# Bardli/RMem_ocu

Hardware: AMD Instinct MI355X
Metric: frames/sec (whole node) 480p VOS, N=8 memory bank (higher is better)
Workload: dtype bf16; 1 GPU; davis17_480p_r50_N8; clip_frames=80, job_clips=64, clip_feeder=static, objects=3, memory_bank=1+7, gap=5, clips_in_flight_per_gpu=24, clips_per_group=8, step_unit=batch, parallelism=clip-parallel x1, weights=synthetic (no checkpoint offline), hipgraphs=True, frames_from=HBM, encoder_lookahead=2

## Files before the change

### include/rmem.h

```cpp
#ifndef RMEM_H_
#define RMEM_H_

#include <stddef.h>

#ifdef __cplusplus
extern "C" {
#endif

#define RMEM_ABI_VERSION 15

int rmem_abi_version(void);
const char* rmem_last_error_string(void);

typedef struct rmem_conv_desc {
  int H, W, Cin;
  int Ho, Wo, Cout;
  int KH, KW, stride, pad;
  int ldo;
  int ldr;
  int ld2;
  int relu;
  int out_f32;
  int res_f32;
  int ldx;
// ... 92 lines not shown
typedef struct rmem_chain_a_desc {
  int L, clips; float eps; int reserved;
  const void* att; float* x;
  const void* w_proj; const float* b_proj; const float* ln2_g; const float* ln2_b; void* curr_v;
  const void* w_q; const float* b_q; void* curr_q;
  const void* short_k; const void* short_v; const float* ln4_g; const float* ln4_b; void* k4; void* v4;
} rmem_chain_a_desc;
int rmem_lstt_chain_a(const rmem_chain_a_desc* d, void* stream);

typedef struct rmem_chain_b_desc {
  int L, clips; float eps; int gn_splits;
  const void* att_long; const void* att_short; float* x;
  const void* w_long; const float* b_long; const void* w_short; const float* b_short; void* tgt3;
  const float* ln3_g; const float* ln3_b; const void* w1; const float* b1; void* h1; float* gn_partial;
} rmem_chain_b_desc;
int rmem_lstt_chain_b(const rmem_chain_b_desc* d, void* stream);

typedef struct rmem_chain_c_desc {
  int L, clips; float eps; int ld_dec;
  float* x;
  const void* h3; const void* w2; const float* b2; const float* dec_g; const float* dec_b; void* dec_out;
  const float* ln1_g; const float* ln1_b; const void* w_qkv; const float* b_qkv; const float* pos_qk; void* qkv;
} rmem_chain_c_desc;
int rmem_lstt_chain_c(const rmem_chain_c_desc* d, void* stream);

int rmem_layernorm(const void* a, int a_is_f32, int lda, const float* gamma, const float* beta, float eps, int M, int C,
                   void* y_bf16, int ldy, float* y_f32, int ldyf, void* stream);

int rmem_patch_merge_ln(const float* x, int H, int W, int C, const float* gamma, const float* beta, float eps,
                        void* y_bf16, void* stream);
int rmem_patch_merge_ln_images(const float* x, int images, int H, int W, int C, const float* gamma, const float* beta, float eps,
                               void* y_bf16, void* stream);

int rmem_window_attn(const void* qkv, const float* qkv_bias, const float* bias_mask_table, void* out, int H, int W,
                     int C, int heads, int shift, void* stream);
int rmem_window_attn_images(const void* qkv, const float* qkv_bias, const float* bias_mask_table, void* out, int images, int H, int W,
                            int C, int heads, int shift, void* stream);

int rmem_add16(const void* a, const void* b, void* y, long long n, void* stream);
int rmem_add16_grouped(int n, const void* const* a, const void* const* b, void* const* y, long long count, void* stream);

size_t rmem_groupnorm_workspace_bytes(int groups);
int rmem_groupnorm_nhwc(const void* x, int M, int C, int groups, const float* gamma, const float* beta,
                        float eps, int act, void* y, float* workspace, void* stream);

int rmem_groupnorm_f32_nhwc(const float* x, int M, int C, int groups, const float* gamma, const float* beta,
                            float eps, int act, void* y, float* workspace, void* stream);

int rmem_groupnorm_nhwc_images(const void* x, int images, int M, int C, int groups, const float* gamma, const float* beta,
                               float eps, int act, void* y, float* workspace, void* stream);
int rmem_groupnorm_head_nhwc_images(const void* x, int images, int M, int C, int groups, const float* gamma, const float* beta,
                                    float eps, int act, const void* w, const float* bias, int N, float* y, int ldy,
                                    float* workspace, void* stream);
int rmem_gn_act_dwconv5x5_nhwc_images(const void* x, int images, int H, int W, int C, int groups, const float* gamma,
                                      const float* beta, float eps, int act, const float* w_t, void* y, float* workspace, void* stream);
int rmem_bilinear_nhwc_images(const void* x, void* y, int images, int Hi, int Wi, int Ho, int Wo, int C, int align_corners, void* stream);
int rmem_gn_act_dwconv5x5_prestats_nhwc_images(const void* x, int images, int H, int W, int C, int groups, const float* gamma,
                                               const float* beta, float eps, int act, const float* w_t, void* y, const float* stats,
                                               void* stream);

int rmem_dwconv5x5_nhwc(const void* x, const float* w_t, void* y, int H, int W, int C, void* stream);

size_t rmem_gated_attn_workspace_bytes(int Lq, int DV, int frames, int keys_per_frame, int nchunks);
int rmem_gated_attn(const void* q, int ldq,
                    const void* k_bank, long long k_slot_stride, int ldk,
                    const void* v_bank, long long v_slot_stride, int ldv,
                    const rmem_attn_chunk* chunks, int nchunks, int frames, int keys_per_frame,
                    const float* pe_cur, const float* pe_mem,
                    int Lq, int DV, const void* u_a, int ldua, const void* u_b, int ldub, int usplit,
                    void* out, int ldo, float* attn_mass,
                    const float* dw_w_t, int H, int W,
                    void* workspace, void* stream);
int rmem_local_gated_attn(const void* q, int ldq, const void* k, int ldk, const void* v, int ldv, const float* rel, int ldrel,
                          int H, int W, int DV, const void* u_a, int ldua, const void* u_b, int ldub, int usplit,
                          void* out, int ldo, const float* dw_w_t, void* workspace, void* stream);

int rmem_gated_attn_clips(const void* q, int ldq, const void* k_bank, long long k_slot_stride, int ldk, const void* v_bank,
                          long long v_slot_stride, int ldv, const rmem_attn_chunk* chunks, int nchunks, int frames, int keys_per_frame,
                          const float* pe_cur, const float* pe_mem, int Lq, int DV, const void* u_a, int ldua, const void* u_b, int ldub,
                          int usplit, void* out, int ldo, float* attn_mass, const float* dw_w_t, int H, int W, int nclips,
                          void* workspace, void* stream);
int rmem_local_gated_attn_clips(const void* q, int ldq, const void* k, int ldk, const void* v, int ldv, const float* rel, int ldrel,
                                int H, int W, int DV, const void* u_a, int ldua, const void* u_b, int ldub, int usplit, void* out, int ldo,
                                const float* dw_w_t, int nclips, void* workspace, void* stream);
int rmem_gated_profile_start(void);
int rmem_gated_profile_stop(double* total_ms, double* total_flops, int* launches);
int rmem_scatter_blocks(const void* src, void* dst, const int* slots_dev, int nclips, long long block_bytes, long long slot_bytes,
                        void* stream);
int rmem_copy2d_async(void* dst, long long dst_pitch, const void* src, long long src_pitch, long long row_bytes, int rows, void* stream);

int rmem_gn_act_dwconv5x5_nhwc(const void* x, int H, int W, int C, int groups, const float* gamma, const float* beta, float eps,
                               int act, const float* w_t, void* y, float* workspace, void* stream);

int rmem_image_to_nhwc8(const float* img_chw, void* out, int H, int W, void* stream);
int rmem_image_to_nhwc8_images(const float* img_chw, void* out, int images, int H, int W, void* stream);
int rmem_image_ptrs_to_nhwc8(const float* const* img_ptrs, void* out, int images, int H, int W, void* stream);
int rmem_stem_padded_size(int H, int W, int* Hp, int* Wp);
int rmem_image_ptrs_to_nhwc4p(const float* const* img_ptrs, void* out_padded, int images, int H, int W, void* stream);
int rmem_stem7x7s2(const void* x_padded, int images, int H, int W, const void* w, const float* bias, void* y, void* stream);
int rmem_stem7x7s2_pool(const void* x_padded, int images, int H, int W, const void* w, const float* bias, void* y_pooled, void* stream);
int rmem_conv3x3_direct(const void* x, int images, int H, int W, int C, const void* w, const float* bias, int relu, void* y, void* stream);
int rmem_conv3x3_c64_direct(const void* x, int images, int H, int W, const void* w, const float* bias, void* y, void* stream);
int rmem_ingest_rgb8(const unsigned char* rgb_hwc, int Hs, int Ws, int Hd, int Wd, float* out_chw, void* out_nhwc8, void* stream);
#define RMEM_JPEG_SUBSEQ_BITS 1024

typedef struct rmem_jpeg_info {
// ... 242 lines not shown
```

### rmem_ocu_amd/_lib.py

```python
from __future__ import annotations

import ctypes as C
import os
import subprocess

_HERE = os.path.dirname(os.path.abspath(__file__))
LIB_PATH = os.environ.get('RMEM_LIB_PATH') or os.path.join(_HERE, 'librmem_hip.so')
ABI_VERSION = 15


class RmemError(RuntimeError):
    pass


class ConvDesc(C.Structure):
    _fields_ = [(n, C.c_int) for n in ('H', 'W', 'Cin', 'Ho', 'Wo', 'Cout', 'KH', 'KW', 'stride', 'pad',
                                       'ldo', 'ldr', 'ld2', 'relu', 'out_f32', 'res_f32', 'ldx', 'batch', 'act_begin',
                                       'res_up_h', 'res_up_w', 'res_up_align')]


class GemmPlan(C.Structure):
    _fields_ = [(n, C.c_int) for n in ('family', 'tile', 'ring', 'is1x1', 'fast', 'splits', 'steps_per_split', 'xcd_ny',
                                       'grid_x', 'grid_y', 'grid_z', 'threads')]

# ... 50 lines not shown
    _fields_ = [('frame', C.c_int), ('value', C.c_int), ('offset', C.c_longlong), ('length', C.c_int)]


class LabelRoute(C.Structure):
    _fields_ = [('dst', C.c_void_p), ('overlay', C.c_void_p), ('feed', C.c_void_p), ('twin', C.c_int), ('mode', C.c_int)]


ROUTE_LIVE, ROUTE_IDLE, ROUTE_SKIP = 0, 1, 2


def _desc(name, ints, ptrs):
    return type(name, (C.Structure,), {'_fields_': [(ints[0], _i), (ints[1], _i), ('eps', _f), (ints[2], _i)] + [(n, _vp) for n in ptrs]})


ChainA = _desc('ChainA', ('L', 'clips', 'reserved'),
               ('att', 'x', 'w_proj', 'b_proj', 'ln2_g', 'ln2_b', 'curr_v', 'w_q', 'b_q', 'curr_q', 'short_k', 'short_v', 'ln4_g', 'ln4_b',
                'k4', 'v4'))
ChainB = _desc('ChainB', ('L', 'clips', 'gn_splits'),
               ('att_long', 'att_short', 'x', 'w_long', 'b_long', 'w_short', 'b_short', 'tgt3', 'ln3_g', 'ln3_b', 'w1', 'b1', 'h1',
                'gn_partial'))
ChainC = _desc('ChainC', ('L', 'clips', 'ld_dec'),
               ('x', 'h3', 'w2', 'b2', 'dec_g', 'dec_b', 'dec_out', 'ln1_g', 'ln1_b', 'w_qkv', 'b_qkv', 'pos_qk', 'qkv'))
SIGNATURES = {
    'rmem_abi_version': (_i, []),
    'rmem_last_error_string': (C.c_char_p, []),
    'rmem_conv_workspace_bytes': (C.c_size_t, [C.POINTER(ConvDesc)]),
    'rmem_conv2d_nhwc': (_i, [C.POINTER(ConvDesc), _vp, _vp, _vp, _vp, _vp, _vp, _vp, _vp]),
    'rmem_conv_plan': (_i, [C.POINTER(ConvDesc), _i, _i, _i, C.POINTER(GemmPlan)]),
    'rmem_attn_workspace_bytes': (C.c_size_t, [_i, _i, _i]),
    'rmem_mem_read_attn': (_i, [_vp, _i, _vp, _vp, _ll, _i, _vp, _i, _i, _vp, _vp, _i, _i, _vp, _i, _vp, _i, _vp, _vp]),
    'rmem_profile_start': (_i, [_i]),
    'rmem_profile_stop': (_i, [C.POINTER(C.c_double), C.POINTER(C.c_double), C.POINTER(_i)]),
    'rmem_layernorm256': (_i, [_vp, _i, _i, _vp, _i, _i, _vp, _vp, _f, _i, _vp, _i, _vp, _vp, _i, _vp, _i, _vp]),
    'rmem_layernorm': (_i, [_vp, _i, _i, _vp, _vp, _f, _i, _i, _vp, _i, _vp, _i, _vp]),
    'rmem_patch_merge_ln': (_i, [_vp, _i, _i, _i, _vp, _vp, _f, _vp, _vp]),
    'rmem_window_attn': (_i, [_vp, _vp, _vp, _vp, _i, _i, _i, _i, _i, _vp]),
    'rmem_window_attn_images': (_i, [_vp, _vp, _vp, _vp, _i, _i, _i, _i, _i, _i, _vp]),
    'rmem_patch_merge_ln_images': (_i, [_vp, _i, _i, _i, _i, _vp, _vp, _f, _vp, _vp]),
    'rmem_add16': (_i, [_vp, _vp, _vp, _ll, _vp]),
    'rmem_add16_grouped': (_i, [_i, C.POINTER(_vp), C.POINTER(_vp), C.POINTER(_vp), _ll, _vp]),
    'rmem_layernorm256_pair': (_i, [_vp, _vp, _vp, _vp, _vp, _vp, _vp, _vp, _f, _i, _vp]),
    'rmem_lstt_chain_waves': (_i, []),
    'rmem_lstt_chain_a': (_i, [C.POINTER(ChainA), _vp]),
    'rmem_lstt_chain_b': (_i, [C.POINTER(ChainB), _vp]),
    'rmem_lstt_chain_c': (_i, [C.POINTER(ChainC), _vp]),
    'rmem_conv1x1_dual_nhwc': (_i, [C.POINTER(ConvDesc), _vp, _vp, _i, _i, _i, _i, _vp, _vp, _vp, _vp]),
    'rmem_bneck_chain': (_i, [C.POINTER(BneckChainDesc), _vp, _vp, _vp, _vp, _vp, _vp, _vp, _vp, _vp, _vp]),
    'rmem_linear_grouped': (_i, [C.POINTER(ConvDesc), _i, C.POINTER(_vp), C.POINTER(_vp), C.POINTER(_vp), C.POINTER(_vp), C.POINTER(_vp), _vp]),
    'rmem_groupnorm_workspace_bytes': (C.c_size_t, [_i]),
    'rmem_groupnorm_nhwc': (_i, [_vp, _i, _i, _i, _vp, _vp, _f, _i, _vp, _vp, _vp]),
    'rmem_groupnorm_f32_nhwc': (_i, [_vp, _i, _i, _i, _vp, _vp, _f, _i, _vp, _vp, _vp]),
    'rmem_groupnorm_nhwc_images': (_i, [_vp, _i, _i, _i, _i, _vp, _vp, _f, _i, _vp, _vp, _vp]),
    'rmem_groupnorm_head_nhwc_images': (_i, [_vp, _i, _i, _i, _i, _vp, _vp, _f, _i, _vp, _vp, _i, _vp, _i, _vp, _vp]),
    'rmem_gn_act_dwconv5x5_nhwc_images': (_i, [_vp, _i, _i, _i, _i, _i, _vp, _vp, _f, _i, _vp, _vp, _vp, _vp]),
    'rmem_gn_act_dwconv5x5_prestats_nhwc_images': (_i, [_vp, _i, _i, _i, _i, _i, _vp, _vp, _f, _i, _vp, _vp, _vp, _vp]),
    'rmem_bilinear_nhwc_images': (_i, [_vp, _vp, _i, _i, _i, _i, _i, _i, _i, _vp]),
    'rmem_mem_read_attn_clips': (_i, [_vp, _i, _vp, _vp, _ll, _i, _vp, _i, _i, _vp, _vp, _i, _i, _vp, _i, _vp, _i, _i, _ll, _ll, _ll, _vp, _vp]),
    'rmem_lstt_attn_pair_clips': (_i, [_vp, _i, _vp, _vp, _ll, _i, _vp, _i, _i, _vp, _vp, _i, _i, _vp, _i, _vp, _i, _i, _ll, _ll,
                                       _vp, _vp, _i, _ll, _vp, _ll, _vp, _vp]),
    'rmem_gn_act_dwconv5x5_nhwc': (_i, [_vp, _i, _i, _i, _i, _vp, _vp, _f, _i, _vp, _vp, _vp, _vp]),
    'rmem_dwconv5x5_nhwc': (_i, [_vp, _vp, _vp, _i, _i, _i, _vp]),
    'rmem_image_to_nhwc8': (_i, [_vp, _vp, _i, _i, _vp]),
    'rmem_image_to_nhwc8_images': (_i, [_vp, _vp, _i, _i, _i, _vp]),
    'rmem_image_ptrs_to_nhwc8': (_i, [_vp, _vp, _i, _i, _i, _vp]),
    'rmem_stem_padded_size': (_i, [_i, _i, C.POINTER(_i), C.POINTER(_i)]),
    'rmem_image_ptrs_to_nhwc4p': (_i, [_vp, _vp, _i, _i, _i, _vp]),
    'rmem_stem7x7s2': (_i, [_vp, _i, _i, _i, _vp, _vp, _vp, _vp]),
    'rmem_stem7x7s2_pool': (_i, [_vp, _i, _i, _i, _vp, _vp, _vp, _vp]),
    'rmem_conv3x3_c64_direct': (_i, [_vp, _i, _i, _i, _vp, _vp, _vp, _vp]),
    'rmem_conv3x3_direct': (_i, [_vp, _i, _i, _i, _i, _vp, _vp, _i, _vp, _vp]),
    'rmem_ingest_rgb8': (_i, [_vp, _i, _i, _i, _i, _vp, _vp, _vp]),
    'rmem_maxpool3x3s2_nhwc': (_i, [_vp, _vp, _i, _i, _i, _vp]),
    'rmem_maxpool3x3s2_nhwc_images': (_i, [_vp, _vp, _i, _i, _i, _i, _vp]),
    'rmem_bilinear_nhwc': (_i, [_vp, _vp, _i, _i, _i, _i, _i, _i, _vp]),
    'rmem_logits_post': (_i, [_vp, _i, _i, _i, _i, _i, _i, _i, _i, _vp, _vp, _vp, _vp]),
    'rmem_logits_post_images': (_i, [_vp, _i, _i, _i, _i, _i, _i, _i, _i, _i, _vp, _vp, _vp, _vp]),
    'rmem_label_to_onehot16': (_i, [_vp, _i, _i, _i, _i, _i, _i, _vp, _vp]),
    'rmem_label_id_embed_scratch_size': (_i, [_i, _i, _i, C.POINTER(_i), C.POINTER(_i)]),
    'rmem_label_id_embed': (_i, [_vp, _i, _i, _i, _i, _i, _i, _i, _i, _i, _i, _i, _vp, _vp, _vp, _vp, _vp]),
    'rmem_label_to_onehot16_images': (_i, [_vp, _i, _i, _i, _i, _i, _i, _i, _vp, _vp]),
    'rmem_evict_scores': (_i, [_vp, _i, _i, _i, _i, _i, _i, _i, _vp, _i, _vp, _vp]),
    'rmem_resize_nearest_flip_f32': (_i, [_vp, _i, _i, _i, _vp, _i, _i, _i, _vp]),
    'rmem_tta_merge': (_i, [C.POINTER(_vp), C.POINTER(_i), _i, _i, _i, _i, _vp, _vp, _vp, _vp]),
    'rmem_logits_post_flip_pairs': (_i, [_vp, _i, _i, _i, _i, _i, _i, _i, _i, _vp, _vp]),
    'rmem_logits_post_ms_merge': (_i, [C.POINTER(_vp), C.POINTER(_i), C.POINTER(_i), C.POINTER(_i), _i, _i, _i, _i, _i, _i, _i, _vp, _vp, _vp]),
    'rmem_route_labels': (_i, [_vp, _i, _i, _i, _vp, _vp]),
    'rmem_label_census': (_i, [_vp, _i, _i, _i, _vp, _vp]),
    'rmem_label_remap': (_i, [_vp, _vp, _i, _ll, _vp, _i, _vp]),
    'rmem_label_pair_census': (_i, [_vp, _vp, _i, _i, _i, _i, _i, _vp, _vp]),
    'rmem_label_pair_census_lds_bins': (_i, []),
    'rmem_mask_iou_counts': (_i, [_vp, _vp, _ll, _i, _i, _vp, _vp]),
    'rmem_clip_score_workspace_bytes': (C.c_size_t, [_i, _i, _i, _i]),
    'rmem_boundary_radius': (_i, [_i, _i, C.c_double]),
    'rmem_clip_score_counts': (_i, [_vp, _vp, _i, _i, _i, _i, _i, _i, _vp, _vp, _vp]),
    'rmem_pair_boundary_workspace_bytes': (C.c_size_t, [_i, _i, _i, _i, _i]),
    'rmem_pair_boundary_counts': (_i, [_vp, _vp, _i, _i, _i, _i, _i, _i, _i, _vp, C.c_size_t, _vp, _vp, _vp, _vp]),
    'rmem_png_zlib_bound': (C.c_size_t, [_i, _i]),
    'rmem_png_workspace_bytes': (C.c_size_t, [_i, _i, _i]),
    'rmem_png_encode_labels': (_i, [_vp, _i, _i, _i, _vp, _vp, _vp, _vp, _vp]),
    'rmem_png_decode_workspace_bytes': (C.c_size_t, [_i, _i, _i]),
    'rmem_png_decode_labels': (_i, [_vp, _vp, _i, _i, _i, _vp, _vp, _vp, _vp, _vp]),
    'rmem_rle_workspace_bytes': (C.c_size_t, [_i, _i, _i, _i]),
    'rmem_rle_encode_labels': (_i, [_vp, _i, _i, _i, _i, _vp, _vp, _ll, _vp, _vp, _vp]),
    'rmem_rle_decode_workspace_bytes': (C.c_size_t, [_ll, _ll, _i, _i]),
    'rmem_rle_decode_labels': (_i, [_vp, _ll, _vp, _i, _i, _i, _i, _vp, _vp, _vp, _vp]),
    'rmem_split_label': (_i, [_vp, _i, _i, _vp, _ll, _vp]),
# ... 73 lines not shown
```

### rmem_ocu_amd/csrc/norm_act.hip

```cpp
#include "common.h"
#include "../../include/rmem.h"

namespace {

struct LnParams {
  const void* a; int a_f32; int lda;
  const void* b; int b_f32; int ldb;
  const float* gamma; const float* beta; float eps; int M;
  e16* y; int ldy; const float* pos; e16* ypos; int ldyp;
  float* yf; int ldyf;
};

__device__ __forceinline__ f32x4 load4(const void* base, int is_f32, long off) {
  if (is_f32) return *reinterpret_cast<const f32x4*>(reinterpret_cast<const float*>(base) + off);
  const e16x4 v = *reinterpret_cast<const e16x4*>(reinterpret_cast<const e16*>(base) + off);
  return f32x4{(float)v[0], (float)v[1], (float)v[2], (float)v[3]};
}

__device__ __forceinline__ void layernorm256_body(const LnParams& p) {
  const int lane = threadIdx.x & 63;
  const int row = blockIdx.x * 4 + (threadIdx.x >> 6);
  if (row >= p.M) return;
  const int c0 = lane * 4;
  f32x4 v = load4(p.a, p.a_f32, (long)row * p.lda + c0);
// ... 254 lines not shown
    for (int j = 0; j < 8; ++j) {
      float f = (d[j] - mean) * rstd * gamma[c0 + j] + beta[c0 + j];
      if (act == 1) f = fmaxf(f, 0.f);
      else if (act == 2) f = gelu_erf(f);
      o[j] = (e16)f;
    }
    reinterpret_cast<e16x8*>(y)[i] = o;
  }
}

template <typename TI>
__global__ __launch_bounds__(256) void k_gn_apply_rows(const TI* x, int M, int C, int cpg, int groups, const float* ws,
                                                       const float* gamma, const float* beta, float eps, int act, e16* y) {
  x += (long)blockIdx.y * M * C;
  y += (long)blockIdx.y * M * C;
  ws += (long)blockIdx.y * groups * GN_SPLITS * 2;
  __shared__ float s_mean[64], s_rstd[64];
  gn_finalize(ws, groups, (float)M * (float)cpg, eps, s_mean, s_rstd);
  __syncthreads();
  constexpr int UN = 8;
  const int vpr = C / 8, rpi = 256 / vpr;
  const int c = threadIdx.x % vpr, rl = threadIdx.x / vpr, c0 = c * 8;
  const float mean = s_mean[c0 / cpg], rstd = s_rstd[c0 / cpg];
  float gm[8], bt[8];
  {
    const f32x4 g0v = *reinterpret_cast<const f32x4*>(gamma + c0), g1v = *reinterpret_cast<const f32x4*>(gamma + c0 + 4);
    const f32x4 b0v = *reinterpret_cast<const f32x4*>(beta + c0), b1v = *reinterpret_cast<const f32x4*>(beta + c0 + 4);
#pragma unroll
    for (int j = 0; j < 4; ++j) { gm[j] = g0v[j]; gm[4 + j] = g1v[j]; bt[j] = b0v[j]; bt[4 + j] = b1v[j]; }
  }
  const int rb = blockIdx.x * (UN * rpi) + rl;
  float d[UN][8];
#pragma unroll
  for (int u = 0; u < UN; ++u) {
    const int r = rb + u * rpi;
    if (r < M) gn_load8(x + (long)r * C + c0, d[u]);
  }
#pragma unroll
  for (int u = 0; u < UN; ++u) {
    const int r = rb + u * rpi;
    if (r >= M) continue;
    e16x8 o;
#pragma unroll
    for (int j = 0; j < 8; ++j) {
      float f = (d[u][j] - mean) * rstd * gm[j] + bt[j];
      if (act == 1) f = fmaxf(f, 0.f);
      else if (act == 2) f = gelu_erf(f);
      o[j] = (e16)f;
    }
    *reinterpret_cast<e16x8*>(y + (long)r * C + c0) = o;
  }
}

constexpr int HC = 128, HPIX = 64, HROW = HC + 8, HPASS = 2;
__global__ __launch_bounds__(256) void k_gn_apply_head(const e16* x, int M, int cpg, int groups, const float* ws, const float* gamma,
                                                       const float* beta, float eps, int act, const e16* w, const float* bias, int N,
                                                       float* y, int ldy) {
  x += (long)blockIdx.y * M * HC;
  y += (long)blockIdx.y * M * ldy;
  ws += (long)blockIdx.y * groups * GN_SPLITS * 2;
  __shared__ float s_mean[64], s_rstd[64];
  __shared__ __attribute__((aligned(16))) e16 tile[HPIX * HROW];
  gn_finalize(ws, groups, (float)M * (float)cpg, eps, s_mean, s_rstd);
  const int tid = threadIdx.x, lane = tid & 63, wave = tid >> 6;
  const int n = lane & 15, kq = lane >> 4;
  e16x8 bf[HC / 32];
#pragma unroll
  for (int ks = 0; ks < HC / 32; ++ks) {
    bf[ks] = e16x8{0, 0, 0, 0, 0, 0, 0, 0};
    if (n < N) bf[ks] = *reinterpret_cast<const e16x8*>(w + n * HC + 32 * ks + 8 * kq);
  }
  const float bn = (bias && n < N) ? bias[n] : 0.f;
  __syncthreads();
  const int c = tid & 15, rl = tid >> 4, c0 = c * 8;
  const float mean = s_mean[c0 / cpg], rstd = s_rstd[c0 / cpg];
  float gm[8], bt[8];
  {
    const f32x4 g0v = *reinterpret_cast<const f32x4*>(gamma + c0), g1v = *reinterpret_cast<const f32x4*>(gamma + c0 + 4);
    const f32x4 b0v = *reinterpret_cast<const f32x4*>(beta + c0), b1v = *reinterpret_cast<const f32x4*>(beta + c0 + 4);
#pragma unroll
    for (int j = 0; j < 4; ++j) { gm[j] = g0v[j]; gm[4 + j] = g1v[j]; bt[j] = b0v[j]; bt[4 + j] = b1v[j]; }
  }
  for (int pass = 0; pass < HPASS; ++pass) {
    const int m0 = (blockIdx.x * HPASS + pass) * HPIX;
    if (m0 >= M) break;
    if (pass > 0) __syncthreads();
    float d[4][8];
#pragma unroll
    for (int u = 0; u < 4; ++u) {
      const int r = m0 + rl + 16 * u;
      if (r < M) gn_load8(x + (long)r * HC + c0, d[u]);
    }
#pragma unroll
    for (int u = 0; u < 4; ++u) {
      const int r = m0 + rl + 16 * u;
      e16x8 o = {0, 0, 0, 0, 0, 0, 0, 0};
      if (r < M) {
#pragma unroll
        for (int j = 0; j < 8; ++j) {
          float f = (d[u][j] - mean) * rstd * gm[j] + bt[j];
          if (act == 1) f = fmaxf(f, 0.f);
          else if (act == 2) f = gelu_erf(f);
          o[j] = (e16)f;
        }
      }
      *reinterpret_cast<e16x8*>(&tile[(rl + 16 * u) * HROW + c0]) = o;
    }
    __syncthreads();
    f32x4 acc = {0.f, 0.f, 0.f, 0.f};
#pragma unroll
    for (int ks = 0; ks < HC / 32; ++ks) {
      const e16x8 a = *reinterpret_cast<const e16x8*>(&tile[(16 * wave + n) * HROW + 32 * ks + 8 * kq]);
      acc = RMEM_MFMA_16x16x32(a, bf[ks], acc, 0, 0, 0);
    }
    if (n < N) {
#pragma unroll
      for (int i = 0; i < 4; ++i) {
        const int m = m0 + 16 * wave + 4 * kq + i;
        if (m < M) y[(long)m * ldy + n] = acc[i] + bn;
      }
    }
  }
}

__global__ __launch_bounds__(256) void k_dwconv5(const e16* x, const float* w, e16* y, int H, int W, int C) {
  const int vpr = C / 8;
  const long total = (long)H * W * vpr;
  const long i = (long)blockIdx.x * 256 + threadIdx.x;
  if (i >= total) return;
  const int c0 = (int)(i % vpr) * 8;
  const int pix = (int)(i / vpr);
  const int py = pix / W, px = pix - py * W;
  float acc[8];
#pragma unroll
  for (int j = 0; j < 8; ++j) acc[j] = 0.f;
  for (int dx = 0; dx < 5; ++dx) {
    const int xx = px + dx - 2;
    if ((unsigned)xx >= (unsigned)W) continue;
    for (int dy = 0; dy < 5; ++dy) {
      const int yy = py + dy - 2;
      if ((unsigned)yy >= (unsigned)H) continue;
      const e16x8 d = *reinterpret_cast<const e16x8*>(x + ((long)yy * W + xx) * C + c0);
      const float* wt = w + (dy * 5 + dx) * C + c0;
      const f32x4 w0 = *reinterpret_cast<const f32x4*>(wt), w1 = *reinterpret_cast<const f32x4*>(wt + 4);
#pragma unroll
      for (int j = 0; j < 4; ++j) { acc[j] += (float)d[j] * w0[j]; acc[4 + j] += (float)d[4 + j] * w1[j]; }
    }
  }
  e16x8 o;
#pragma unroll
  for (int j = 0; j < 8; ++j) o[j] = (e16)acc[j];
  reinterpret_cast<e16x8*>(y)[i] = o;
}

constexpr int DT_H = 8, DT_W = 16, DT_C = 64, DT_HW = (DT_H + 4) * (DT_W + 4);
__global__ __launch_bounds__(256) void k_gn_dwconv5(const e16* x, const float* ws, const float* gamma, const float* beta, float eps,
                                                    int cpg, int act, const float* w, e16* y, int H, int W, int C, int M) {
  __shared__ __attribute__((aligned(16))) e16 tile[DT_HW * DT_C];
  __shared__ __attribute__((aligned(16))) float wl[25 * DT_C];
  __shared__ float s_mean[8], s_rstd[8];
  const int tid = threadIdx.x;
// ... 174 lines not shown
  const int blocks = (int)min((long)1024, (n8 + 255) / 256);
  hipLaunchKernelGGL(k_add16_grouped, dim3(blocks, n), dim3(256), 0, (hipStream_t)stream, g, n8);
  return rmem_check_launch("rmem_add16_grouped");
}

namespace {
template <typename TI>
void gn_launch_stats(const TI* x, int images, int M, int C, int cpg, float* ws, hipStream_t s) {
  const int vpr = C / 8;
  if (vpr <= 256 && 256 % vpr == 0)
    hipLaunchKernelGGL(k_gn_stats_rows<TI>, dim3(GN_SPLITS, 1, images), dim3(256), 0, s, x, M, C, cpg, ws);
  else
    hipLaunchKernelGGL(k_gn_stats<TI>, dim3(C / cpg, GN_SPLITS, images), dim3(256), 0, s, x, M, C, cpg, ws);
}
template <typename TI>
void gn_launch_apply(const TI* x, int images, int M, int C, int cpg, const float* ws, const float* gamma, const float* beta, float eps,
                     int act, e16* y, hipStream_t s) {
  const int vpr = C / 8, groups = C / cpg;
  if (vpr <= 256 && 256 % vpr == 0) {
    const int rows_per_wg = 8 * (256 / vpr);
    hipLaunchKernelGGL(k_gn_apply_rows<TI>, dim3((M + rows_per_wg - 1) / rows_per_wg, images), dim3(256), 0, s, x, M, C, cpg, groups, ws,
                       gamma, beta, eps, act, y);
  } else {
    const long total = (long)M * vpr;
    const int blocks = (int)min((long)2048, (total + 255) / 256);
    hipLaunchKernelGGL(k_gn_apply<TI>, dim3(blocks, images), dim3(256), 0, s, x, M, C, cpg, groups, ws, gamma, beta, eps, act, y);
  }
}
}

#ifndef RMEM_F16
extern "C" size_t rmem_groupnorm_workspace_bytes(int groups) { return (size_t)groups * GN_SPLITS * 2 * sizeof(float); }
#endif

static int gn_check(const void* x, const void* y, const float* gamma, const float* beta, const float* ws, int groups, int C, int act,
                    int M, int images) {
  RMEM_REQUIRE(x && y && gamma && beta && ws, "rmem_groupnorm: null argument");
  RMEM_REQUIRE(groups >= 1 && groups <= 64 && C % groups == 0 && (C / groups) % 8 == 0,
               "rmem_groupnorm: channels per group must be a multiple of 8 and groups <= 64");
  RMEM_REQUIRE(act >= 0 && act <= 2 && M > 0 && images >= 1, "rmem_groupnorm: bad act / M / images");
  return 0;
}

extern "C" int RMEM_API(rmem_groupnorm_nhwc_images)(const void* x, int images, int M, int C, int groups, const float* gamma, const float* beta,
                                          float eps, int act, void* y, float* workspace, void* stream) {
  if (gn_check(x, y, gamma, beta, workspace, groups, C, act, M, images)) return -1;
  const int cpg = C / groups;
  hipStream_t s = (hipStream_t)stream;
  gn_launch_stats((const e16*)x, images, M, C, cpg, workspace, s);
  gn_launch_apply((const e16*)x, images, M, C, cpg, workspace, gamma, beta, eps, act, (e16*)y, s);
  return rmem_check_launch("rmem_groupnorm_nhwc_images");
}

extern "C" int RMEM_API(rmem_groupnorm_head_nhwc_images)(const void* x, int images, int M, int C, int groups, const float* gamma, const float* beta,
                                               float eps, int act, const void* w, const float* bias, int N, float* y, int ldy,
                                               float* workspace, void* stream) {
  if (gn_check(x, y, gamma, beta, workspace, groups, C, act, M, images)) return -1;
  RMEM_REQUIRE(C == 128 && w && N >= 1 && N <= 16 && ldy >= N, "rmem_groupnorm_head_nhwc: C must be 128, 1 <= N <= 16 <= ... ldy >= N");
  RMEM_REQUIRE((uintptr_t)w % 16 == 0, "rmem_groupnorm_head_nhwc: w must be 16-byte aligned");
  const int cpg = C / groups;
  hipStream_t s = (hipStream_t)stream;
  gn_launch_stats((const e16*)x, images, M, C, cpg, workspace, s);
  hipLaunchKernelGGL(k_gn_apply_head, dim3((M + HPIX * HPASS - 1) / (HPIX * HPASS), images), dim3(256), 0, s, (const e16*)x, M, cpg, groups, workspace, gamma,
                     beta, eps, act, (const e16*)w, bias, N, y, ldy);
  return rmem_check_launch("rmem_groupnorm_head_nhwc_images");
}

extern "C" int RMEM_API(rmem_groupnorm_nhwc)(const void* x, int M, int C, int groups, const float* gamma, const float* beta, float eps,
                                   int act, void* y, float* workspace, void* stream) {
  RMEM_REQUIRE(x && y && gamma && beta && workspace, "rmem_groupnorm_nhwc: null argument");
  RMEM_REQUIRE(groups >= 1 && groups <= 64 && C % groups == 0 && (C / groups) % 8 == 0,
               "rmem_groupnorm_nhwc: channels per group must be a multiple of 8 and groups <= 64");
  RMEM_REQUIRE(act >= 0 && act <= 2 && M > 0, "rmem_groupnorm_nhwc: bad act / M");
  const int cpg = C / groups;
  hipStream_t s = (hipStream_t)stream;
  gn_launch_stats((const e16*)x, 1, M, C, cpg, workspace, s);
  gn_launch_apply((const e16*)x, 1, M, C, cpg, workspace, gamma, beta, eps, act, (e16*)y, s);
  return rmem_check_launch("rmem_groupnorm_nhwc");
}

extern "C" int RMEM_API(rmem_groupnorm_f32_nhwc)(const float* x, int M, int C, int groups, const float* gamma, const float* beta, float eps,
                                       int act, void* y, float* workspace, void* stream) {
  RMEM_REQUIRE(x && y && gamma && beta && workspace, "rmem_groupnorm_f32_nhwc: null argument");
  RMEM_REQUIRE(groups >= 1 && groups <= 64 && C % groups == 0 && (C / groups) % 8 == 0,
               "rmem_groupnorm_f32_nhwc: groups must divide C into multiples of 8 channels (<= 64 groups)");
  RMEM_REQUIRE(act >= 0 && act <= 2 && M > 0, "rmem_groupnorm_f32_nhwc: bad act / M");
  const int cpg = C / groups;
  hipStream_t s = (hipStream_t)stream;
  gn_launch_stats(x, 1, M, C, cpg, workspace, s);
  gn_launch_apply(x, 1, M, C, cpg, workspace, gamma, beta, eps, act, (e16*)y, s);
  return rmem_check_launch("rmem_groupnorm_f32_nhwc");
}

extern "C" int RMEM_API(rmem_gn_act_dwconv5x5_nhwc_images)(const void* x, int images, int H, int W, int C, int groups, const float* gamma,
                                                 const float* beta, float eps, int act, const float* w_t, void* y, float* workspace,
                                                 void* stream);
extern "C" int RMEM_API(rmem_gn_act_dwconv5x5_nhwc)(const void* x, int H, int W, int C, int groups, const float* gamma, const float* beta,
                                          float eps, int act, const float* w_t, void* y, float* workspace, void* stream) {
  return RMEM_API(rmem_gn_act_dwconv5x5_nhwc_images)(x, 1, H, W, C, groups, gamma, beta, eps, act, w_t, y, workspace, stream);
}

static int gn_act_dwconv_launch(const void* x, int images, int H, int W, int C, int groups, const float* gamma, const float* beta, float eps,
                                int act, const float* w_t, void* y, float* workspace, void* stream, bool with_stats);
extern "C" int RMEM_API(rmem_gn_act_dwconv5x5_nhwc_images)(const void* x, int images, int H, int W, int C, int groups, const float* gamma,
                                                 const float* beta, float eps, int act, const float* w_t, void* y, float* workspace,
                                                 void* stream) {
  return gn_act_dwconv_launch(x, images, H, W, C, groups, gamma, beta, eps, act, w_t, y, workspace, stream, true);
}
extern "C" int RMEM_API(rmem_gn_act_dwconv5x5_prestats_nhwc_images)(const void* x, int images, int H, int W, int C, int groups, const float* gamma,
                                                          const float* beta, float eps, int act, const float* w_t, void* y,
                                                          const float* stats, void* stream) {
  return gn_act_dwconv_launch(x, images, H, W, C, groups, gamma, beta, eps, act, w_t, y, const_cast<float*>(stats), stream, false);
}
static int gn_act_dwconv_launch(const void* x, int images, int H, int W, int C, int groups, const float* gamma, const float* beta, float eps,
                                int act, const float* w_t, void* y, float* workspace, void* stream, bool with_stats) {
  RMEM_REQUIRE(images >= 1, "rmem_gn_act_dwconv5x5_nhwc: images must be >= 1");
  RMEM_REQUIRE(x && y && gamma && beta && w_t && workspace && H > 0 && W > 0, "rmem_gn_act_dwconv5x5_nhwc: bad argument");
// ... 19 lines not shown
```

### rmem_ocu_amd/csrc/resample.hip

```cpp
#include "common.h"
#include "../../include/rmem.h"

namespace {

__global__ __launch_bounds__(256) void k_image_to_nhwc8(const float* img, e16* out, int H, int W) {
  const long n = (long)H * W;
  const long i = (long)blockIdx.x * 256 + threadIdx.x;
  if (i >= n) return;
  img += (long)blockIdx.y * 3 * n;
  out += (long)blockIdx.y * 8 * n;
  e16x8 o = {0, 0, 0, 0, 0, 0, 0, 0};
  o[0] = (e16)img[i];
  o[1] = (e16)img[n + i];
  o[2] = (e16)img[2 * n + i];
  reinterpret_cast<e16x8*>(out)[i] = o;
}

__global__ __launch_bounds__(256) void k_image_ptrs_to_nhwc8(const float* const* imgs, e16* out, int H, int W) {
  const long n = (long)H * W;
  const long i = (long)blockIdx.x * 256 + threadIdx.x;
  if (i >= n) return;
  const float* img = imgs[blockIdx.y];
  out += (long)blockIdx.y * 8 * n;
  e16x8 o = {0, 0, 0, 0, 0, 0, 0, 0};
// ... 82 lines not shown
    src_coord(ox, Wi, Wo, align, x0, x1, wx);
    if (x0 != cx0 || x1 != cx1) {
      const float* a = lg + ((long)y0 * Wi + x0) * 16;
      const float* b = lg + ((long)y0 * Wi + x1) * 16;
      const float* c = lg + ((long)y1 * Wi + x0) * 16;
      const float* d = lg + ((long)y1 * Wi + x1) * 16;
#pragma unroll
      for (int q = 0; q < 4; ++q) {
        const f32x4 ta = *reinterpret_cast<const f32x4*>(a + 4 * q), tb = *reinterpret_cast<const f32x4*>(b + 4 * q);
        const f32x4 tc = *reinterpret_cast<const f32x4*>(c + 4 * q), td = *reinterpret_cast<const f32x4*>(d + 4 * q);
#pragma unroll
        for (int j = 0; j < 4; ++j) { va[4 * q + j] = ta[j]; vb[4 * q + j] = tb[j]; vc[4 * q + j] = tc[j]; vd[4 * q + j] = td[j]; }
      }
      cx0 = x0; cx1 = x1;
    }
    float best = -3.0e38f; int arg = 0;
#pragma unroll
    for (int ch = 0; ch < 16; ++ch) {
      if (ch < nc) {
        float v;
        if (ch > keep) v = -1.0e10f;
        else {
          const float top = va[ch] * (1.f - wx) + vb[ch] * wx;
          const float bot = vc[ch] * (1.f - wx) + vd[ch] * wx;
          v = top * (1.f - wy) + bot * wy;
        }
        if (v > best) { best = v; arg = ch; }
      }
    }
    const long i = (long)oy * Wo + ox;
    if (label) label[i] = (uint8_t)arg;
    if (label_f32) label_f32[i] = (float)arg;
  }
}

constexpr int LT_H = 16, LT_W = 64, LT_SRC = 12 * 40;
__global__ __launch_bounds__(256) void k_logits_labels_tile(const float* lg, int nc, int keep, int Hi, int Wi, int Ho, int Wo, int align,
                                                            uint8_t* label, float* label_f32) {
  __shared__ __attribute__((aligned(16))) float src[LT_SRC * 16];
  const int tiles_x = (Wo + LT_W - 1) / LT_W;
  const int ty = blockIdx.x / tiles_x, tx = blockIdx.x - ty * tiles_x;
  const long total = (long)Ho * Wo;
  lg += (long)blockIdx.y * Hi * Wi * 16;
  if (label) label += (long)blockIdx.y * total;
  if (label_f32) label_f32 += (long)blockIdx.y * total;
  const int oy0 = ty * LT_H, ox0 = tx * LT_W;
  const int oy1 = min(oy0 + LT_H, Ho) - 1, ox1 = min(ox0 + LT_W, Wo) - 1;
  int ylo, yhi, xlo, xhi, t0, t1; float tw;
  src_coord(oy0, Hi, Ho, align, ylo, t1, tw);
  src_coord(oy1, Hi, Ho, align, t0, yhi, tw);
  src_coord(ox0, Wi, Wo, align, xlo, t1, tw);
  src_coord(ox1, Wi, Wo, align, t0, xhi, tw);
  const int ncols = xhi - xlo + 1, nrows = yhi - ylo + 1;
  for (int i = threadIdx.x; i < nrows * ncols * 4; i += 256) {
    const int pix = i >> 2, q = i & 3;
    const int r = pix / ncols, c = pix - r * ncols;
    *reinterpret_cast<f32x4*>(&src[pix * 16 + 4 * q]) = *reinterpret_cast<const f32x4*>(lg + ((long)(ylo + r) * Wi + xlo + c) * 16 + 4 * q);
  }
  __syncthreads();
  const int oy = oy0 + (threadIdx.x >> 4), oxb = ox0 + (threadIdx.x & 15) * 4;
  if (oy >= Ho) return;
  int y0, y1; float wy;
  src_coord(oy, Hi, Ho, align, y0, y1, wy);
#pragma unroll
  for (int k = 0; k < 4; ++k) {
    const int ox = oxb + k;
    if (ox >= Wo) break;
    int x0, x1; float wx;
    src_coord(ox, Wi, Wo, align, x0, x1, wx);
    const float* a = &src[((y0 - ylo) * ncols + (x0 - xlo)) * 16];
    const float* b = &src[((y0 - ylo) * ncols + (x1 - xlo)) * 16];
    const float* c = &src[((y1 - ylo) * ncols + (x0 - xlo)) * 16];
    const float* d = &src[((y1 - ylo) * ncols + (x1 - xlo)) * 16];
    float best = -3.0e38f; int arg = 0;
#pragma unroll
    for (int q = 0; q < 4; ++q) {
      const f32x4 ta = *reinterpret_cast<const f32x4*>(a + 4 * q), tb = *reinterpret_cast<const f32x4*>(b + 4 * q);
      const f32x4 tc = *reinterpret_cast<const f32x4*>(c + 4 * q), td = *reinterpret_cast<const f32x4*>(d + 4 * q);
#pragma unroll
      for (int j = 0; j < 4; ++j) {
        const int ch = 4 * q + j;
        if (ch < nc) {
          float v;
          if (ch > keep) v = -1.0e10f;
          else {
            const float top = ta[j] * (1.f - wx) + tb[j] * wx;
            const float bot = tc[j] * (1.f - wx) + td[j] * wx;
            v = top * (1.f - wy) + bot * wy;
          }
          if (v > best) { best = v; arg = ch; }
        }
      }
    }
    const long i = (long)oy * Wo + ox;
    if (label) label[i] = (uint8_t)arg;
    if (label_f32) label_f32[i] = (float)arg;
  }
}

bool lt_tiles_fit(int Hi, int Wi, int Ho, int Wo, int align) {
  int rows = 0, cols = 0, lo, hi, t; float w;
  for (int o0 = 0; o0 < Ho; o0 += LT_H) {
    rmem_src_coord(o0, Hi, Ho, align, lo, t, w);
    rmem_src_coord((o0 + LT_H < Ho ? o0 + LT_H : Ho) - 1, Hi, Ho, align, t, hi, w);
    rows = hi - lo + 1 > rows ? hi - lo + 1 : rows;
  }
  for (int o0 = 0; o0 < Wo; o0 += LT_W) {
    rmem_src_coord(o0, Wi, Wo, align, lo, t, w);
    rmem_src_coord((o0 + LT_W < Wo ? o0 + LT_W : Wo) - 1, Wi, Wo, align, t, hi, w);
    cols = hi - lo + 1 > cols ? hi - lo + 1 : cols;
  }
  return rows * cols <= LT_SRC;
}

__global__ __launch_bounds__(256) void k_logits_post(const float* lg, int ldl, int nc, int keep, int Hi, int Wi, int Ho, int Wo,
                                                     int align, float* out, uint8_t* label, float* label_f32) {
  const long total = (long)Ho * Wo;
  const long i = (long)blockIdx.x * 256 + threadIdx.x;
  if (i >= total) return;
  lg += (long)blockIdx.y * Hi * Wi * ldl;
  if (label) label += (long)blockIdx.y * total;
  if (label_f32) label_f32 += (long)blockIdx.y * total;
  const int oy = (int)(i / Wo), ox = (int)(i - (long)oy * Wo);
  int y0, y1, x0, x1; float wy, wx;
  src_coord(oy, Hi, Ho, align, y0, y1, wy);
  src_coord(ox, Wi, Wo, align, x0, x1, wx);
  const float* a = lg + ((long)y0 * Wi + x0) * ldl;
  const float* b = lg + ((long)y0 * Wi + x1) * ldl;
  const float* c = lg + ((long)y1 * Wi + x0) * ldl;
  const float* d = lg + ((long)y1 * Wi + x1) * ldl;
  float best = -3.0e38f; int arg = 0;
  if (ldl == 16 && !out) {
    float va[16], vb[16], vc[16], vd[16];
#pragma unroll
    for (int q = 0; q < 4; ++q) {
      const f32x4 ta = *reinterpret_cast<const f32x4*>(a + 4 * q), tb = *reinterpret_cast<const f32x4*>(b + 4 * q);
      const f32x4 tc = *reinterpret_cast<const f32x4*>(c + 4 * q), td = *reinterpret_cast<const f32x4*>(d + 4 * q);
#pragma unroll
      for (int j = 0; j < 4; ++j) { va[4 * q + j] = ta[j]; vb[4 * q + j] = tb[j]; vc[4 * q + j] = tc[j]; vd[4 * q + j] = td[j]; }
    }
#pragma unroll
    for (int ch = 0; ch < 16; ++ch) {
      if (ch < nc) {
        float v;
        if (ch > keep) v = -1.0e10f;
        else {
// ... 708 lines not shown
```

Before: 3322 frames/s.

## Prefetch next GN-head rows, raise passes per block, skip unused logit channels

The fused groupnorm-head kernel now register-prefetches the next 64-row tile while the current tile's matmul runs, and loads the first tile before the stats finalize. Passes per block go from 2 to 8, and the activation becomes a template parameter so the per-element branch disappears. Separately, the logits-to-labels kernel only loads and scans the 4-channel groups up to the kept object index, which cuts shared-memory traffic when there are few objects. The higher pass count gives fewer blocks, which can hurt occupancy, and the prefetch adds register pressure.

```diff
diff --git a/include/rmem.h b/include/rmem.h
--- a/include/rmem.h
+++ b/include/rmem.h
@@ -168,6 +168,7 @@
 int rmem_groupnorm_head_nhwc_images(const void* x, int images, int M, int C, int groups, const float* gamma, const float* beta,
                                     float eps, int act, const void* w, const float* bias, int N, float* y, int ldy,
                                     float* workspace, void* stream);
+int rmem_groupnorm_head_rows(void);
 int rmem_gn_act_dwconv5x5_nhwc_images(const void* x, int images, int H, int W, int C, int groups, const float* gamma,
                                       const float* beta, float eps, int act, const float* w_t, void* y, float* workspace, void* stream);
 int rmem_bilinear_nhwc_images(const void* x, void* y, int images, int Hi, int Wi, int Ho, int Wo, int C, int align_corners, void* stream);
diff --git a/rmem_ocu_amd/_lib.py b/rmem_ocu_amd/_lib.py
--- a/rmem_ocu_amd/_lib.py
+++ b/rmem_ocu_amd/_lib.py
@@ -126,6 +126,7 @@
     'rmem_groupnorm_f32_nhwc': (_i, [_vp, _i, _i, _i, _vp, _vp, _f, _i, _vp, _vp, _vp]),
     'rmem_groupnorm_nhwc_images': (_i, [_vp, _i, _i, _i, _i, _vp, _vp, _f, _i, _vp, _vp, _vp]),
     'rmem_groupnorm_head_nhwc_images': (_i, [_vp, _i, _i, _i, _i, _vp, _vp, _f, _i, _vp, _vp, _i, _vp, _i, _vp, _vp]),
+    'rmem_groupnorm_head_rows': (_i, []),
     'rmem_gn_act_dwconv5x5_nhwc_images': (_i, [_vp, _i, _i, _i, _i, _i, _vp, _vp, _f, _i, _vp, _vp, _vp, _vp]),
     'rmem_gn_act_dwconv5x5_prestats_nhwc_images': (_i, [_vp, _i, _i, _i, _i, _i, _vp, _vp, _f, _i, _vp, _vp, _vp, _vp]),
     'rmem_bilinear_nhwc_images': (_i, [_vp, _vp, _i, _i, _i, _i, _i, _i, _i, _vp]),
diff --git a/rmem_ocu_amd/csrc/norm_act.hip b/rmem_ocu_amd/csrc/norm_act.hip
--- a/rmem_ocu_amd/csrc/norm_act.hip
+++ b/rmem_ocu_amd/csrc/norm_act.hip
@@ -330,17 +330,28 @@
   }
 }
 
-constexpr int HC = 128, HPIX = 64, HROW = HC + 8, HPASS = 2;
+#ifndef RMEM_HEAD_PASSES
+#define RMEM_HEAD_PASSES 8
+#endif
+constexpr int HC = 128, HPIX = 64, HROW = HC + 8, HPASS = RMEM_HEAD_PASSES;
+template <int ACT>
 __global__ __launch_bounds__(256) void k_gn_apply_head(const e16* x, int M, int cpg, int groups, const float* ws, const float* gamma,
-                                                       const float* beta, float eps, int act, const e16* w, const float* bias, int N,
+                                                       const float* beta, float eps, const e16* w, const float* bias, int N,
                                                        float* y, int ldy) {
   x += (long)blockIdx.y * M * HC;
   y += (long)blockIdx.y * M * ldy;
   ws += (long)blockIdx.y * groups * GN_SPLITS * 2;
   __shared__ float s_mean[64], s_rstd[64];
   __shared__ __attribute__((aligned(16))) e16 tile[HPIX * HROW];
+  const int tid = threadIdx.x, lane = tid & 63, wave = tid >> 6;
+  const int c = tid & 15, rl = tid >> 4, c0 = c * 8;
+  e16x8 raw[4];
+  auto load_rows = [&](int m0) {
+#pragma unroll
+    for (int u = 0; u < 4; ++u) raw[u] = *reinterpret_cast<const e16x8*>(x + (long)min(m0 + rl + 16 * u, M - 1) * HC + c0);
+  };
+  load_rows(blockIdx.x * HPASS * HPIX);
   gn_finalize(ws, groups, (float)M * (float)cpg, eps, s_mean, s_rstd);
-  const int tid = threadIdx.x, lane = tid & 63, wave = tid >> 6;
   const int n = lane & 15, kq = lane >> 4;
   e16x8 bf[HC / 32];
 #pragma unroll
@@ -350,7 +361,6 @@
   }
   const float bn = (bias && n < N) ? bias[n] : 0.f;
   __syncthreads();
-  const int c = tid & 15, rl = tid >> 4, c0 = c * 8;
   const float mean = s_mean[c0 / cpg], rstd = s_rstd[c0 / cpg];
   float gm[8], bt[8];
   {
@@ -363,12 +373,6 @@
     const int m0 = (blockIdx.x * HPASS + pass) * HPIX;
     if (m0 >= M) break;
     if (pass > 0) __syncthreads();
-    float d[4][8];
-#pragma unroll
-    for (int u = 0; u < 4; ++u) {
-      const int r = m0 + rl + 16 * u;
-      if (r < M) gn_load8(x + (long)r * HC + c0, d[u]);
-    }
 #pragma unroll
     for (int u = 0; u < 4; ++u) {
       const int r = m0 + rl + 16 * u;
@@ -376,15 +380,16 @@
       if (r < M) {
 #pragma unroll
         for (int j = 0; j < 8; ++j) {
-          float f = (d[u][j] - mean) * rstd * gm[j] + bt[j];
-          if (act == 1) f = fmaxf(f, 0.f);
-          else if (act == 2) f = gelu_erf(f);
+          float f = ((float)raw[u][j] - mean) * rstd * gm[j] + bt[j];
+          if (ACT == 1) f = fmaxf(f, 0.f);
+          else if (ACT == 2) f = gelu_erf(f);
           o[j] = (e16)f;
         }
       }
       *reinterpret_cast<e16x8*>(&tile[(rl + 16 * u) * HROW + c0]) = o;
     }
     __syncthreads();
+    if (pass + 1 < HPASS) load_rows(m0 + HPIX);
     f32x4 acc = {0.f, 0.f, 0.f, 0.f};
 #pragma unroll
     for (int ks = 0; ks < HC / 32; ++ks) {
@@ -665,6 +670,10 @@
   return rmem_check_launch("rmem_groupnorm_nhwc_images");
 }
 
+#ifndef RMEM_F16
+extern "C" int rmem_groupnorm_head_rows(void) { return HPIX * HPASS; }
+#endif
+
 extern "C" int RMEM_API(rmem_groupnorm_head_nhwc_images)(const void* x, int images, int M, int C, int groups, const float* gamma, const float* beta,
                                                float eps, int act, const void* w, const float* bias, int N, float* y, int ldy,
                                                float* workspace, void* stream) {
@@ -674,8 +683,9 @@
   const int cpg = C / groups;
   hipStream_t s = (hipStream_t)stream;
   gn_launch_stats((const e16*)x, images, M, C, cpg, workspace, s);
-  hipLaunchKernelGGL(k_gn_apply_head, dim3((M + HPIX * HPASS - 1) / (HPIX * HPASS), images), dim3(256), 0, s, (const e16*)x, M, cpg, groups, workspace, gamma,
-                     beta, eps, act, (const e16*)w, bias, N, y, ldy);
+  const auto kern = act == 1 ? k_gn_apply_head<1> : act == 2 ? k_gn_apply_head<2> : k_gn_apply_head<0>;
+  hipLaunchKernelGGL(kern, dim3((M + HPIX * HPASS - 1) / (HPIX * HPASS), images), dim3(256), 0, s, (const e16*)x, M, cpg, groups, workspace, gamma,
+                     beta, eps, (const e16*)w, bias, N, y, ldy);
   return rmem_check_launch("rmem_groupnorm_head_nhwc_images");
 }
 
diff --git a/rmem_ocu_amd/csrc/resample.hip b/rmem_ocu_amd/csrc/resample.hip
--- a/rmem_ocu_amd/csrc/resample.hip
+++ b/rmem_ocu_amd/csrc/resample.hip
@@ -158,10 +158,12 @@
   src_coord(ox0, Wi, Wo, align, xlo, t1, tw);
   src_coord(ox1, Wi, Wo, align, t0, xhi, tw);
   const int ncols = xhi - xlo + 1, nrows = yhi - ylo + 1;
+  const int nq = max(min(keep, nc - 1), 0) / 4 + 1;
   for (int i = threadIdx.x; i < nrows * ncols * 4; i += 256) {
     const int pix = i >> 2, q = i & 3;
     const int r = pix / ncols, c = pix - r * ncols;
-    *reinterpret_cast<f32x4*>(&src[pix * 16 + 4 * q]) = *reinterpret_cast<const f32x4*>(lg + ((long)(ylo + r) * Wi + xlo + c) * 16 + 4 * q);
+    if (q < nq)
+      *reinterpret_cast<f32x4*>(&src[pix * 16 + 4 * q]) = *reinterpret_cast<const f32x4*>(lg + ((long)(ylo + r) * Wi + xlo + c) * 16 + 4 * q);
   }
   __syncthreads();
   const int oy = oy0 + (threadIdx.x >> 4), oxb = ox0 + (threadIdx.x & 15) * 4;
@@ -181,6 +183,7 @@
     float best = -3.0e38f; int arg = 0;
 #pragma unroll
     for (int q = 0; q < 4; ++q) {
+      if (q >= nq) break;
       const f32x4 ta = *reinterpret_cast<const f32x4*>(a + 4 * q), tb = *reinterpret_cast<const f32x4*>(b + 4 * q);
       const f32x4 tc = *reinterpret_cast<const f32x4*>(c + 4 * q), td = *reinterpret_cast<const f32x4*>(d + 4 * q);
 #pragma unroll
@@ -198,6 +201,7 @@
         }
       }
     }
+    if (4 * nq < nc && -1.0e10f > best) arg = 4 * nq;
     const long i = (long)oy * Wo + ox;
     if (label) label[i] = (uint8_t)arg;
     if (label_f32) label_f32[i] = (float)arg;
```

Measured after the change: 3322 frames/s, median of 2. About the same (+0.0%).
